# muonzoo/cutesdr

Measured on AMD Instinct MI355X. Metric: complex IQ MSamples/s through CFastFIR+demod chain; achieved HBM GB/s vs peak, higher is better.
Workload: dtype f32; 1 GPU; C3: 256 channels/GPU x 2^19 IQ samples, 16384-pt CFastFIR overlap-save (8193 taps, hop 8192), shared -5..+5 kHz filter @62.5 kS/s; channels_per_gpu=256, samples_per_channel=524288, fft_size=16384, parallelism=channels sharded x1, no data-path collective

## Files before the change

cutesdr_amd/csrc/capi_fastfir.hip:

```cpp
#include "capi_common.hpp"
#include "capi_internal.hpp"
#include <algorithm>
#include "fastfir_kernels.h"
#include "fastfir_design_kernels.h"
#include "host_math.hpp"
#include "patch_queue.hpp"
#include <cmath>
#include <cstdlib>
#include <cstring>
#include <vector>

using namespace csdr;

static int log2_of(int n)
{
    int l = 0;
    while ((1 << l) < n) l++;
    return ((1 << l) == n) ? l : -1;
}

struct csdr_fastfir_batch {
    int device, channels, n, log2n;
    int cus;
    hipStream_t last_stream;
// ... 60 lines not shown
            if (e == hipSuccess) e = hipEventRecord(b->ev_design, s);
        }
    }
    const int rr = b->patches.retire(s);
    if (rc) return rc;
    if (e != hipSuccess) return fail(CSDR_EHIP, "filter design launch: %s", hipGetErrorString(e));
    return rr;
}

static int fetch_mirror(csdr_fastfir_batch *b, int slot)
{
    if (!b->stale[slot]) return CSDR_OK;
    const int rc = flush_control(b, b->last_stream);
    if (rc) return rc;
    if (b->ev_design) CSDR_HIP(hipEventSynchronize(b->ev_design));
    CSDR_HIP(hipMemcpy(b->resp[slot].data(), b->d_resp + (size_t)slot * 2 * b->n, sizeof(cd) * (size_t)b->n, hipMemcpyDeviceToHost));
    b->stale[slot] = 0;
    return CSDR_OK;
}

static int design_state(csdr_fastfir_batch *b)
{
    if (b->d_resp) return CSDR_OK;
    const size_t n = (size_t)b->n, p = n / 2 + 1;
    const auto win = fastfir_window((int)p);
    const auto tw = design_twiddles(n);
    if (!b->d_win) CSDR_HIP(hipMalloc((void **)&b->d_win, p * sizeof(double)));
    if (!b->d_tw) CSDR_HIP(hipMalloc((void **)&b->d_tw, n * sizeof(double)));
    if (!b->d_perm) CSDR_HIP(hipMalloc((void **)&b->d_perm, n * sizeof(int)));
    if (!b->d_perm2) CSDR_HIP(hipMalloc((void **)&b->d_perm2, n * sizeof(int)));
    if (!b->d_permg) CSDR_HIP(hipMalloc((void **)&b->d_permg, n * sizeof(int)));
    CSDR_HIP(hipMemcpy(b->d_win, win->data(), p * sizeof(double), hipMemcpyHostToDevice));
    CSDR_HIP(hipMemcpy(b->d_tw, tw.data(), n * sizeof(double), hipMemcpyHostToDevice));
    CSDR_HIP(hipMemcpy(b->d_perm, b->perm.data(), n * sizeof(int), hipMemcpyHostToDevice));
    CSDR_HIP(hipMemcpy(b->d_perm2, b->perm2.data(), n * sizeof(int), hipMemcpyHostToDevice));
    CSDR_HIP(hipMemcpy(b->d_permg, b->permg.data(), n * sizeof(int), hipMemcpyHostToDevice));
    CSDR_HIP(hipMalloc((void **)&b->d_resp, (size_t)b->channels * n * sizeof(cd)));
    return CSDR_OK;
}

static void build_perm(csdr_fastfir_batch *b)
{
    const int T = b->n / 32;
    b->perm.resize(b->n);
    for (int j = 0; j < 16; j++)
        for (int t = 0; t < T; t++)
            for (int e = 0; e < 2; e++)
                b->perm[(j * T + t) * 2 + e] = fastfir_bin_of(b->log2n, t, 2 * j + e);
    b->perm2.clear();
    {
        b->perm2.resize(b->n);
        for (int j = 0; j < 16; j++)
            for (int t = 0; t < T; t++)
                for (int e = 0; e < 2; e++) b->perm2[(j * T + t) * 2 + e] = fastfir2_bin_of(b->log2n, t, j, e);
    }
    b->permg.resize(b->n);
    for (int i = 0; i < 8; i++)
        for (int t = 0; t < T; t++)
            for (int c = 0; c < 4; c++) b->permg[(i * T + t) * 4 + c] = fastfir2_gain_bin_of(b->log2n, t, i, c);
}

static int upload_response(csdr_fastfir_batch *b, int slot, const std::vector<cd> &H)
{
    std::vector<float> dev(2 * (size_t)b->n);
    for (int pass = 0; pass < 2; pass++) {
        const std::vector<int> &perm = pass ? b->perm2 : b->perm;
        float *dst = pass ? b->d_h2 : b->d_h;
        if (perm.empty() || !dst) continue;
        for (int i = 0; i < b->n; i++) {
            const cd v = H[perm[i]];
            dev[2 * i] = (float)v.real();
            dev[2 * i + 1] = (float)v.imag();
        }
        const int rc = b->patches.add(dst + (size_t)slot * 2 * b->n, dev.data(), dev.size() * sizeof(float));
        if (rc) return rc;
    }
    for (int i = 0; i < b->n; i++) dev[i] = (float)fastfir_gain(H[b->permg[i]], b->permg[i]);
    return b->patches.add(b->d_gain + (size_t)slot * b->n, dev.data(), (size_t)b->n * sizeof(float));
}

static int set_response(csdr_fastfir_batch *b, int slot, const std::vector<cd> &H)
{
    cancel_job(b, slot);
    const int rc = upload_response(b, slot, H);
    if (rc) return rc;
    b->resp[slot] = H;
    b->stale[slot] = 0;
    return CSDR_OK;
}

extern "C" {

csdr_fastfir_batch *csdr_fastfir_batch_create(int device, int channels, int fft_size)
{
    const int l2 = log2_of(fft_size);
    if (l2 < 11 || l2 > 14 || channels < 1) {
        fail(CSDR_EINVAL, "fft_size must be 2048..16384 (power of two), channels >= 1");
        return nullptr;
    }
    if (!device_ok(device)) return nullptr;
    csdr_fastfir_batch *b = new csdr_fastfir_batch();
    b->device = device; b->channels = channels; b->n = fft_size; b->log2n = l2;
    b->per_channel = false; b->hist_cur = 0; b->dbg_stage = 0; b->dbg_out = nullptr;
    b->last_stream = nullptr;
    {
        int cus = 0;
        if (hipDeviceGetAttribute(&cus, hipDeviceAttributeMultiprocessorCount, device) != hipSuccess || cus <= 0) cus = 256;
        b->cus = cus;
    }
    {
        const char *v = getenv("CSDR_FASTFIR_VARIANT");
        b->variant = (v && atoi(v) == 0) ? 0 : 2;
// ... 358 lines not shown
```

cutesdr_amd/csrc/capi_hosttest.hip:

```cpp
#include "capi_common.hpp"
#include "host_math.hpp"
#include "dc_host.hpp"
#include "pc_host.hpp"
#include "display_plan.hpp"
#include "testgen_host.hpp"
#include "scope_host.hpp"
#include "fastfir_kernels.h"
#include "fft_core.hpp"
#include <cstring>

using namespace csdr;

template <int SIGN> static void host_head4_gain(const float *x4, const float *g4, float *out4)
{
    v2f x[4];
    for (int q = 0; q < 4; q++) x[q] = v2f{x4[2 * q], x4[2 * q + 1]};
    dit_head4_gain<0, 4, SIGN>(x, v2f{g4[0], g4[1]}, v2f{g4[2], g4[3]});
    for (int q = 0; q < 4; q++) { out4[2 * q] = x[q].x; out4[2 * q + 1] = x[q].y; }
}
template <int R, int SIGN> static void host_dft_middle(const float *in, float *out)
{
    v2f x[R];
    for (int n = 0; n < R; n++) x[bitrev<R>(n)] = v2f{in[2 * n], in[2 * n + 1]};
    static_for<0, R / 4>([&](auto G) { dit_head4<G.value, R, SIGN>(x); });
    if constexpr (R == 32) dit_single<8, 32, SIGN>(x);
    static_for<0, R / 4>([&](auto I) { dit_tail_middle<I.value, R, SIGN>(x); });
    for (int r = 0; r < R / 2; r++) { out[2 * r] = x[R / 4 + r].x; out[2 * r + 1] = x[R / 4 + r].y; }
}

extern "C" {

int csdr__host_fastfir_design(int n, double flo, double fhi, double off, double fs, double *h_out)
{
    std::vector<cd> H;
    if (!fastfir_design(n, flo, fhi, off, fs, H)) return -1;
    memcpy(h_out, H.data(), sizeof(cd) * n);
    return 0;
}
int csdr__host_design_job(double flo, double fhi, double off, double fs, double *nfc, double *nfs)
{
    return fastfir_design_job(flo, fhi, off, fs, *nfc, *nfs) ? 0 : -1;
}
int csdr__host_fastfir_bin_of(int log2n, int t, int r) { return fastfir_bin_of(log2n, t, r); }
int csdr__host_fastfir_gains(int n, double flo, double fhi, double off, double fs, double *h_out, double *p_out)
{
    std::vector<cd> H;
    if (!fastfir_design(n, flo, fhi, off, fs, H)) return -1;
    memcpy(h_out, H.data(), sizeof(cd) * n);
    for (int k = 0; k < n; k++) p_out[k] = fastfir_gain(H[k], k);
    return 0;
}
int csdr__host_fastfir2_bin_of(int log2n, int t, int j, int e) { return fastfir2_bin_of(log2n, t, j, e); }
int csdr__host_fastfir2_gain_bin_of(int log2n, int t, int i, int c) { return fastfir2_gain_bin_of(log2n, t, i, c); }

void csdr__host_dit_head4_gain(int sign, const float *x4, const float *g4, float *out4)
{
    if (sign > 0) host_head4_gain<+1>(x4, g4, out4); else host_head4_gain<-1>(x4, g4, out4);
}
int csdr__host_dft_middle(int r, int sign, const float *in, float *out)
{
    if (r == 16 && sign > 0) host_dft_middle<16, +1>(in, out);
    else if (r == 16) host_dft_middle<16, -1>(in, out);
    else if (r == 32 && sign > 0) host_dft_middle<32, +1>(in, out);
    else if (r == 32) host_dft_middle<32, -1>(in, out);
    else return -1;
    return 0;
}

int csdr__host_dc_plan(double in_rate, double bw, int *codes, double *out_rate, int *warmup)
{
    DcPlan p = dc_make_plan(in_rate, bw);
    for (int i = 0; i < p.nstages; i++) codes[i] = p.kind[i];
    *out_rate = p.out_rate; *warmup = p.W;
    return p.nstages;
}
int csdr__host_dc_stage_taps(double in_rate, double bw, int s, double *h)
{
    DcPlan p = dc_make_plan(in_rate, bw);
    if (s < 0 || s >= p.nstages) return -1;
    const DcStage &st = p.st[s];
    const int L = st.hist + (p.kind[s] == 3 ? 2 : 1);
    for (int i = 0; i < L; i++) h[i] = 0;
    if (st.center >= 0) h[st.center] = st.ccoef;
    for (int q = 0; q < st.npairs; q++) { h[st.a[q]] = st.c[q]; h[st.b[q]] = st.c[q]; }
    return L;
}
void csdr__host_dc_nco(double freq, double cw, double in_rate, unsigned long long *inc, double *stored)
{
    DcHostChan c;
    c.in_rate = in_rate; c.cw_offset = cw;
    c.set_frequency(freq);
    *inc = c.inc; *stored = c.nco_freq;
}
int csdr__host_fir_design(int kind, double scale, double astop, double fpass, double fstop, double fs,
                          double hilbert_off, double *coef, double *icoef, double *qcoef)
{
    HostFir f;
    if (kind == 0) f.init_lp(scale, astop, fpass, fstop, fs);
    else f.init_hp(scale, astop, fpass, fstop, fs);
    if (hilbert_off != 0.0) f.gen_hilbert(hilbert_off);
    for (int i = 0; i < f.ntaps; i++) { coef[i] = f.coef[i]; icoef[i] = f.icoef[i]; qcoef[i] = f.qcoef[i]; }
    return f.ntaps;
}
void csdr__host_iir_design(int kind, double f0, double q, double fs, double *c5)
{
    PcIir f;
// ... 185 lines not shown
```

cutesdr_amd/csrc/fastfir2_kernels.hip:

```cpp
#define CSDR_FMA_BFLY 1
#define CSDR_PLAIN_CONST_FMA 1
#include "launch_once.hpp"
#include "fastfir_dev.hpp"
#include "fastfir_kernels.h"

namespace csdr {

#define CSDR_SB() __builtin_amdgcn_sched_barrier(0)

#ifndef K1_LDAUX
#define K1_LDAUX 2
#endif
#ifndef K1_STAUX
#define K1_STAUX 2
#endif
#ifndef K1_HREG
#define K1_HREG 8
#endif
#ifndef K1_REALGAIN
#define K1_REALGAIN 1
#endif
#ifndef K1_TWREG
#define K1_TWREG 0
#endif
#ifndef K1_HREG4K
#define K1_HREG4K 4
#endif
#ifndef K1_W1_FETCH_MAX_R0
#define K1_W1_FETCH_MAX_R0 2
#endif
#ifndef K1_HREG2K
#define K1_HREG2K 8
#endif

#ifdef CSDR_K1_STAMPS
#define CSDR_STAMP(i)                                                                         \
    do {                                                                                      \
        CSDR_SB();                                                                            \
        unsigned long long now_;                                                              \
        asm volatile("s_memtime %0\n\ts_waitcnt lgkmcnt(0)" : "=s"(now_)::"memory");         \
        CSDR_SB();                                                                            \
        acc_[i] += now_ - last_;                                                              \
        last_ = now_;                                                                         \
    } while (0)
#else
#define CSDR_STAMP(i) do { } while (0)
#endif

#define CSDR_PRIO(p) __builtin_amdgcn_s_setprio(p)

#ifdef K1_ABLATE
__device__ __forceinline__ void keep_alive(v4f v) { asm volatile("" ::"v"(v)); }
#endif

template <int LOG2N>
struct K1Cfg {
    using Base = FastFirCfg<LOG2N>;
    static constexpr int VW = LOG2N == 12 ? 2 : (LOG2N == 11 ? 4 : 1);
    static constexpr int TV = Base::T;
    static constexpr int T = VW * TV;
    static constexpr int LDS_BYTES = (VW * Base::LDS_DATA + 1024) * 8;
};

template <int LOG2N, bool RG>
__device__ __forceinline__ void fastfir_os2_body(const FastFirArgs a)
{
    CSDR_WG_TRACE_SCOPE(a.trace, WGT_FF);
    static_assert(!RG || LOG2N == 14, "the quarter-block shift is whole rows of the outer pass at N = 16384 only");
    using Cfg = FastFirCfg<LOG2N>;
    constexpr int N = Cfg::N, T = Cfg::T, R0 = Cfg::R0, G = Cfg::G, L = N / 2;
    constexpr int HALF = R0 / 2;
    constexpr int VW = K1Cfg<LOG2N>::VW;
    constexpr int HREG = RG ? 0 : (LOG2N == 12 ? K1_HREG4K : (LOG2N == 11 ? K1_HREG2K : K1_HREG));
    constexpr int TWREG = RG ? K1_TWREG : 0;
    static_assert(R0 == 16 || R0 == 8 || R0 == 4 || R0 == 2, "the grouped outer pass is written for N = 2048 ... 16384");
    auto block_barrier = [] {
        if constexpr (LOG2N == 11) {
            __builtin_amdgcn_fence(__ATOMIC_RELEASE, "wavefront"); __builtin_amdgcn_wave_barrier(); __builtin_amdgcn_fence(__ATOMIC_ACQUIRE, "wavefront");
        } else {
            __syncthreads();
        }
    };
    extern __shared__ __attribute__((aligned(16))) unsigned char smem_raw[];
    const int t = VW == 1 ? (int)threadIdx.x : (int)threadIdx.x % T, vw = VW == 1 ? 0 : (int)threadIdx.x / T;
    v2f *lds = reinterpret_cast<v2f *>(smem_raw) + vw * Cfg::LDS_DATA;
    v2f *tw2 = reinterpret_cast<v2f *>(smem_raw) + VW * Cfg::LDS_DATA;
    if constexpr (VW > 1) {
        for (int i = threadIdx.x; i < 1024; i += VW * T) tw2[i] = a.tw2[i];
        __syncthreads();
    }

    int wg = blockIdx.x * VW + vw, ch, run;
    if ((a.channels & 7) == 0) {
        int xcd = wg & 7, slot = wg >> 3;
        ch = (slot / a.runs) * 8 + xcd;
        run = slot % a.runs;
    } else {
        ch = wg / a.runs;
        run = wg % a.runs;
    }
    const int b0 = run * a.blocks_per_run;
    int b1 = b0 + a.blocks_per_run;
    if (b1 > a.nblocks) b1 = a.nblocks;
#if defined(__HIP_DEVICE_COMPILE__) && !defined(__gfx950__)
#error "fastfir_os2_kernel<12> relies on gfx950's s_barrier ignoring terminated waves (two virtual workgroups per workgroup)"
#endif
    if (ch >= a.channels || b0 >= b1) return;

    if constexpr (VW == 1)
        for (int i = t; i < 1024; i += T) tw2[i] = a.tw2[i];

    const rsrc_t r_in = make_rsrc(a.in + (long)ch * a.in_stride, (unsigned)a.nblocks * L * 8u);
    const rsrc_t r_hist = make_rsrc(a.hist + (long)ch * L, L * 8u);
    const rsrc_t r_out = make_rsrc(a.out + (long)ch * a.out_stride, (unsigned)a.nblocks * L * 8u);
    const rsrc_t r_h = make_rsrc(a.h + (long)ch * a.h_stride, N * 8u);
    const rsrc_t r_g = make_rsrc(a.gain + (long)ch * (a.h_stride / 2), N * 4u);
    constexpr int PSTEP = 2 * T, PSTEP_LDS = PSTEP + 2 * (PSTEP / 32), PSTEP_B = PSTEP * 8;
    const int voff = t * 16;
    auto load_half = [&](rsrc_t r, int soff, v2f (&dst)[16]) {
#pragma unroll
        for (int n1 = 0; n1 < HALF; n1++)
#pragma unroll
            for (int pp = 0; pp < G / 2; pp++) {
                v4f v = buf_load16_aux<K1_LDAUX>(r, voff + pp * PSTEP_B, soff + n1 * 8192);
                dst[(2 * pp) * HALF + n1] = v2f{v.x, v.y};
                dst[(2 * pp + 1) * HALF + n1] = v2f{v.z, v.w};
            }
    };

    constexpr bool W1_RESIDENT = R0 > K1_W1_FETCH_MAX_R0;
    auto w_pair = [&](int pp) { return *reinterpret_cast<const v4f *>(a.tw1 + PSTEP * pp + 2 * t); };
    v2f w1[R0 > 2 ? G : 1];
    auto load_w1 = [&] {
        if constexpr (R0 > 2) {
#pragma unroll
            for (int pp = 0; pp < G / 2; pp++) { const v4f v = w_pair(pp); w1[2 * pp] = v2f{v.x, v.y}; w1[2 * pp + 1] = v2f{v.z, v.w}; }
        }
    };
    load_w1();
    v2f pw[G][R0];
    if constexpr (R0 > 2) {
#pragma unroll
        for (int e = 0; e < G; e++) twiddle_powers<R0>(opaque(w1[e]), pw[e]);
    }

    v4f hv[RG ? 1 : 16];
#pragma unroll
    for (int j = 0; j < HREG; j++) hv[j] = buf_load16(r_h, t * 16, j * (T * 16));
    v4f pv[RG ? 8 : 1];
    if constexpr (RG) {
#pragma unroll
        for (int i = 0; i < 8; i++) pv[i] = buf_load16(r_g, t * 16, i * (T * 16));
    }
#ifdef K1_ABLATE
    v4f habl = {1.0f, 0.0f, 1.0f, 0.0f};
    asm volatile("" : "+v"(habl));
    v2f twabl = {0.8f, 0.6f};
    asm volatile("" : "+v"(twabl));
#endif
    v2f x[32];
    v2f hp[16], hq[16];

    if (b0 == 0) load_half(r_hist, 0, hp);
    else load_half(r_in, (b0 - 1) * (L * 8), hp);
    load_half(r_in, b0 * (L * 8), hq);

    const int sb = t >> 5, sn = t & 31;
    v2f *const col = lds + lds_pad(1024 * sb) + sn;
    const v2f *const twc = tw2 + sn;
    v2f twr[TWREG > 0 ? TWREG : 1];
#pragma unroll
    for (int k1 = 1; k1 <= TWREG; k1++) twr[k1 - 1] = a.tw2[32 * k1 + sn];
    auto pass_tw = [&](auto K1) {
        constexpr int k1 = K1.value;
        if constexpr (k1 <= TWREG) return twr[k1 - 1];
        else return lds_ld8(twc + 32 * k1);
    };
    v2f *const rowp = lds + 34 * t;
    v2f *const outer = lds + lds_pad(2 * t);
    constexpr int OUTER_ROW = 1024 + 2 * (1024 / 32);

#ifdef K1_CYC
    const unsigned long long cyc0_ = __builtin_amdgcn_s_memtime(), rt0_ = __builtin_amdgcn_s_memrealtime();
#endif
#ifdef CSDR_K1_STAMPS
    unsigned long long acc_[16] = {0, 0, 0, 0, 0, 0, 0, 0, 0, 0, 0, 0, 0, 0, 0, 0}, last_;
    asm volatile("s_memtime %0\n\ts_waitcnt lgkmcnt(0)" : "=s"(last_)::"memory");
#endif
    auto one_block = [&](const int b, v2f (&oldh)[16], v2f (&newh)[16]) {
        CSDR_SB();
        CSDR_PRIO(1);
        {
            v2f y[G][R0];
            static_for<0, HALF>([&](auto N1) {
                static_for<0, G>([&](auto E) {
                    constexpr int e = E.value, n1 = N1.value, po = bitrev<R0>(n1), pn = bitrev<R0>(HALF + n1);
                    y[e][po] = oldh[e * HALF + n1]; y[e][pn] = newh[e * HALF + n1];
                });
            });
            if constexpr (R0 == 2) {
                static_for<0, G>([&](auto E) { bfly_dit<0, +1>(y[E.value][0], y[E.value][1]); });
            } else {
                static_for<0, (R0 >= 8 ? R0 / 4 : 1)>([&](auto Gg) {
                    static_for<0, G>([&](auto E) { dit_head4<Gg.value, R0, +1>(y[E.value]); });
                });
            }
            CSDR_SB();
            load_half(r_in, (b + 1 < a.nblocks ? b + 1 : a.nblocks - 1) * (L * 8), oldh);
            CSDR_SB();
            CSDR_PRIO(0);
            v4f wv[16];
            if constexpr (R0 == 16) {
                static_for<0, R0 / 4 + 1>([&](auto Ii) {
                    constexpr int i = Ii.value;
                    if constexpr (i < R0 / 4) {
                        dit_tail<i, R0, +1>(y[0]);
                        dit_tail<i, R0, +1>(y[1]);
                        static_for<0, 4>([&](auto P) {
                            constexpr int k0 = i + 4 * P.value;
                            if constexpr (k0 != 0) {
                                y[0][k0] = cmul(y[0][k0], pw[0][k0]);
                                y[1][k0] = cmul(y[1][k0], pw[1][k0]);
                            }
                            wv[k0] = store_operand(y[0][k0], y[1][k0]);
                        });
                    }
                    if constexpr (i > 0) {
                        CSDR_STORE_GROUP_BEGIN();
                        static_for<0, 4>([&](auto P) {
                            constexpr int k0 = (i - 1) + 4 * P.value;
                            *reinterpret_cast<v4f *>(outer + OUTER_ROW * k0) = wv[k0];
                        });
                        CSDR_STORE_GROUP_END();
                    } else {
                        CSDR_SB();
                    }
                });
            } else if constexpr (R0 == 2) {
                v4f wq[8];
                static_for<0, 8>([&](auto PP) { wq[PP.value] = w_pair(PP.value); });
                static_for<0, 5>([&](auto Ii) {
                    constexpr int i = Ii.value;
                    if constexpr (i < 4) {
                        static_for<0, 2>([&](auto Q) {
                            constexpr int pp = 2 * i + Q.value;
                            y[2 * pp][1] = cmul(y[2 * pp][1], v2f{wq[pp].x, wq[pp].y});
                            y[2 * pp + 1][1] = cmul(y[2 * pp + 1][1], v2f{wq[pp].z, wq[pp].w});
                            wv[pp] = store_operand(y[2 * pp][0], y[2 * pp + 1][0]);
                            wv[8 + pp] = store_operand(y[2 * pp][1], y[2 * pp + 1][1]);
                        });
                    }
                    if constexpr (i > 0) {
                        CSDR_STORE_GROUP_BEGIN();
                        static_for<0, 2>([&](auto Q) {
                            constexpr int pp = 2 * (i - 1) + Q.value;
                            *reinterpret_cast<v4f *>(outer + PSTEP_LDS * pp) = wv[pp];
                            *reinterpret_cast<v4f *>(outer + OUTER_ROW + PSTEP_LDS * pp) = wv[8 + pp];
                        });
                        CSDR_STORE_GROUP_END();
                    } else {
                        CSDR_SB();
                    }
                });
            } else {
                constexpr int NG = 4, RPG = R0 / NG;
                static_for<0, NG + 1>([&](auto Ii) {
                    constexpr int i = Ii.value;
                    if constexpr (i < NG) {
                        if constexpr (R0 == 8)
                            static_for<0, G>([&](auto E) { bfly_dit<4 * i, +1>(y[E.value][i], y[E.value][i + 4]); });
                        static_for<0, RPG>([&](auto P) {
                            constexpr int k0 = i + NG * P.value;
                            static_for<0, G>([&](auto E) {
                                if constexpr (k0 != 0) y[E.value][k0] = cmul(y[E.value][k0], pw[E.value][k0]);
                            });
                            static_for<0, G / 2>([&](auto PP) {
                                wv[k0 * (G / 2) + PP.value] = store_operand(y[2 * PP.value][k0], y[2 * PP.value + 1][k0]);
                            });
                        });
                    }
                    if constexpr (i > 0) {
                        CSDR_STORE_GROUP_BEGIN();
                        static_for<0, RPG>([&](auto P) {
                            constexpr int k0 = (i - 1) + NG * P.value;
                            static_for<0, G / 2>([&](auto PP) {
                                *reinterpret_cast<v4f *>(outer + OUTER_ROW * k0 + PSTEP_LDS * PP.value) = wv[k0 * (G / 2) + PP.value];
                            });
                        });
                        CSDR_STORE_GROUP_END();
                    } else {
                        CSDR_SB();
                    }
                });
            }
        }
        CSDR_STAMP(0);
#ifdef ABL_BAR
        __builtin_amdgcn_fence(__ATOMIC_RELEASE, "wavefront"); __builtin_amdgcn_wave_barrier(); __builtin_amdgcn_fence(__ATOMIC_ACQUIRE, "wavefront");
#else
        block_barrier();
#endif
        CSDR_STAMP(1);

        CSDR_PRIO(3);
        {
            auto fetch = [&](auto Gg) {
                static_for<0, 4>([&](auto Q) {
                    constexpr int p = 4 * Gg.value + Q.value;
                    x[p] = lds_ld8(col + 34 * bitrev<32>(p));
                });
            };
            static_for<0, 3>(fetch);
            CSDR_SB();
            static_for<0, 8>([&](auto Gg) {
                if constexpr (Gg.value + 3 < 8) fetch(std::integral_constant<int, Gg.value + 3>{});
                dit_head4<Gg.value, 32, +1>(x);
                if constexpr ((Gg.value & 1) == 1) CSDR_SB();
            });
            CSDR_STAMP(7);
            dit_single<8, 32, +1>(x);
            CSDR_SB();
            v2f tw[2][4];
#ifdef ABL_TW
            static_for<1, 4>([&](auto P) { tw[0][P.value] = twabl; });
#else
            static_for<1, 4>([&](auto P) { tw[0][P.value] = pass_tw(std::integral_constant<int, 8 * P.value>{}); });
#endif
            CSDR_SB();
            CSDR_STAMP(8);
            static_for<0, 9>([&](auto Ii) {
                constexpr int i = Ii.value;
                if constexpr (i < 7)
#ifdef ABL_TW
                    static_for<0, 4>([&](auto P) { tw[(i + 1) & 1][P.value] = twabl; });
#else
                    static_for<0, 4>([&](auto P) { tw[(i + 1) & 1][P.value] = pass_tw(std::integral_constant<int, i + 1 + 8 * P.value>{}); });
#endif
                if constexpr (i < 8) {
#ifdef ABL_H
                    if constexpr (!RG) { hv[2 * i] = habl; hv[2 * i + 1] = habl; }
#else
                    if constexpr (!RG && 2 * i >= HREG) hv[2 * i] = buf_load16(r_h, t * 16, (2 * i) * (T * 16));
                    if constexpr (!RG && 2 * i + 1 >= HREG) hv[2 * i + 1] = buf_load16(r_h, t * 16, (2 * i + 1) * (T * 16));
#endif
                    dit_tail<i, 32, +1>(x);
                    static_for<0, 4>([&](auto P) {
                        constexpr int k1 = i + 8 * P.value;
                        if constexpr (k1 != 0) x[k1] = cmul(x[k1], tw[i & 1][P.value]);
                    });
                }
                if constexpr (i > 0)
                    static_for<0, 4>([&](auto P) {
                        constexpr int k1 = (i - 1) + 8 * P.value;
                        lds_st8(col + 34 * k1, x[k1]);
                    });
                CSDR_SB();
            });
        }
        CSDR_STAMP(2);
        __builtin_amdgcn_fence(__ATOMIC_RELEASE, "wavefront");
        __builtin_amdgcn_wave_barrier();
        __builtin_amdgcn_fence(__ATOMIC_ACQUIRE, "wavefront");

        CSDR_PRIO(2);
        {
            v2f y[32];
            static_for<0, 4>([&](auto Q) {
                static_for<0, 4>([&](auto P) {
                    constexpr int j = Q.value + 4 * P.value;
                    const v4f v = *reinterpret_cast<const v4f *>(rowp + 2 * j);
                    x[bitrev<32>(2 * j)] = v2f{v.x, v.y};
                    x[bitrev<32>(2 * j + 1)] = v2f{v.z, v.w};
                });
            });
            CSDR_SB();
            static_for<0, 4>([&](auto Q) {
                dit_head4<bitrev<8>(2 * Q.value), 32, +1>(x);
                dit_head4<bitrev<8>(2 * Q.value + 1), 32, +1>(x);
                CSDR_SB();
            });
            dit_single<8, 32, +1>(x);
            CSDR_SB();
            static_for<0, 8>([&](auto Ii) {
                constexpr int i = Ii.value, g = bitrev<8>(i);
                dit_tail<i, 32, +1>(x);
                y[4 * g] = x[i]; y[4 * g + 1] = x[i + 16]; y[4 * g + 2] = x[i + 8]; y[4 * g + 3] = x[i + 24];
                if constexpr (RG)
                    dit_head4_gain<g, 32, -1>(y, v2f{pv[i].x, pv[i].y}, v2f{pv[i].z, pv[i].w});
                else
                    dit_head4_tw<g, 32, -1>(y, v2f{hv[2 * i].x, hv[2 * i].y}, v2f{hv[2 * i].z, hv[2 * i].w},
                                            v2f{hv[2 * i + 1].x, hv[2 * i + 1].y}, v2f{hv[2 * i + 1].z, hv[2 * i + 1].w});
                if constexpr ((i & 1) == 1) CSDR_SB();
            });
#pragma unroll
            for (int i = 0; i < 32; i++) x[i] = y[i];
            CSDR_PRIO(1);
            dit_single<8, 32, -1>(x);
            CSDR_SB();
            v4f wv[16];
            static_for<0, 5>([&](auto Q) {
                constexpr int q = Q.value;
                if constexpr (q < 4) {
                    dit_tail<2 * q, 32, -1>(x);
                    dit_tail<2 * q + 1, 32, -1>(x);
                    static_for<0, 4>([&](auto P) {
                        constexpr int j = q + 4 * P.value;
                        wv[j] = store_operand(x[2 * j], x[2 * j + 1]);
                    });
                }
                if constexpr (q > 0) {
                    CSDR_STORE_GROUP_BEGIN();
                    static_for<0, 4>([&](auto P) {
                        constexpr int j = (q - 1) + 4 * P.value;
                        *reinterpret_cast<v4f *>(rowp + 2 * j) = wv[j];
                    });
                    CSDR_STORE_GROUP_END();
                } else {
                    CSDR_SB();
                }
            });
        }
        CSDR_STAMP(3);
        __builtin_amdgcn_fence(__ATOMIC_RELEASE, "wavefront");
        __builtin_amdgcn_wave_barrier();
        __builtin_amdgcn_fence(__ATOMIC_ACQUIRE, "wavefront");

        CSDR_PRIO(0);
        {
            v2f tw[32];
            auto fetch = [&](auto Gg) {
                static_for<0, 4>([&](auto Q) {
                    constexpr int r = 4 * Gg.value + Q.value;
                    x[r] = lds_ld8(col + 34 * bitrev<32>(r));
                });
                static_for<0, 4>([&](auto Q) {
                    constexpr int r = 4 * Gg.value + Q.value;
#ifdef ABL_TW
                    if constexpr (r != 0) tw[r] = twabl;
#else
                    if constexpr (r != 0) tw[r] = pass_tw(std::integral_constant<int, bitrev<32>(r)>{});
#endif
                });
            };
            static_for<0, 2>(fetch);
            CSDR_SB();
            static_for<0, 8>([&](auto Gg) {
                constexpr int g = Gg.value;
                if constexpr (g + 2 < 8) fetch(std::integral_constant<int, g + 2>{});
                dit_head4_conjtw<g, 32, -1, g == 0>(x, tw[4 * g], tw[4 * g + 1], tw[4 * g + 2], tw[4 * g + 3]);
                if constexpr ((g & 1) == 1) CSDR_SB();
            });
            dit_single<8, 32, -1>(x);
            CSDR_SB();
            static_for<0, 9>([&](auto I) {
                constexpr int i = I.value;
                if constexpr (i < 8) dit_tail<i, 32, -1>(x);
                if constexpr (i > 0)
                    static_for<0, 4>([&](auto P) {
                        constexpr int n1 = (i - 1) + 8 * P.value;
                        lds_st8(col + 34 * n1, x[n1]);
                    });
                CSDR_SB();
            });
        }
        CSDR_STAMP(4);
#ifdef ABL_BAR
        __builtin_amdgcn_fence(__ATOMIC_RELEASE, "wavefront"); __builtin_amdgcn_wave_barrier(); __builtin_amdgcn_fence(__ATOMIC_ACQUIRE, "wavefront");
#else
        block_barrier();
#endif
        CSDR_STAMP(5);

        CSDR_PRIO(3);
        {
            v2f y[G][R0];
            static_for<0, R0>([&](auto Rr) {
                constexpr int r = Rr.value, k0 = bitrev<R0>(r);
                static_for<0, G / 2>([&](auto PP) {
                    const v4f v = *reinterpret_cast<const v4f *>(outer + OUTER_ROW * k0 + PSTEP_LDS * PP.value);
                    y[2 * PP.value][r] = v2f{v.x, v.y};
                    y[2 * PP.value + 1][r] = v2f{v.z, v.w};
                });
            });
            if constexpr (R0 > 2) {
                if constexpr (!W1_RESIDENT) load_w1();
#pragma unroll
                for (int e = 0; e < G; e++) twiddle_powers<R0>(opaque(w1[e]), pw[e]);
                CSDR_SB();
                static_for<0, (R0 >= 8 ? R0 / 4 : 1)>([&](auto Gg) {
                    constexpr int g = Gg.value;
                    static_for<0, G>([&](auto E) {
                        constexpr int e = E.value;
                        dit_head4_conjtw<g, R0, -1, g == 0>(y[e], pw[e][bitrev<R0>(4 * g)], pw[e][bitrev<R0>(4 * g + 1)],
                                                            pw[e][bitrev<R0>(4 * g + 2)], pw[e][bitrev<R0>(4 * g + 3)]);
                    });
                    if constexpr ((g & 1) == 1) CSDR_SB();
                });
            }
            CSDR_PRIO(2);
            v4f sv[8];
            if constexpr (R0 == 16) {
                static_for<0, R0 / 4 + 1>([&](auto I) {
                    constexpr int i = I.value;
                    if constexpr (i < R0 / 4) {
                        if constexpr (RG) {
                            dit_tail_middle<i, R0, -1>(y[0]);
                            dit_tail_middle<i, R0, -1>(y[1]);
                            sv[2 * i] = store_operand(y[0][i + 4], y[1][i + 4]);
                            sv[2 * i + 1] = store_operand(y[0][i + 8], y[1][i + 8]);
                        } else {
                            dit_tail_upper<i, R0, -1>(y[0]);
                            dit_tail_upper<i, R0, -1>(y[1]);
                            sv[2 * i] = store_operand(y[0][i + 8], y[1][i + 8]);
                            sv[2 * i + 1] = store_operand(y[0][i + 12], y[1][i + 12]);
                        }
                    }
                    if constexpr (i > 0) {
                        CSDR_STORE_GROUP_BEGIN();
#ifdef ABL_GST
                        keep_alive(sv[2 * (i - 1)]); keep_alive(sv[2 * (i - 1) + 1]);
#else
                        buf_store16_aux<K1_STAUX>(r_out, voff, b * (L * 8) + (i - 1) * 8192, sv[2 * (i - 1)]);
                        buf_store16_aux<K1_STAUX>(r_out, voff, b * (L * 8) + (i - 1 + 4) * 8192, sv[2 * (i - 1) + 1]);
#endif
                        CSDR_STORE_GROUP_END();
                    } else {
                        CSDR_SB();
                    }
                });
            } else if constexpr (R0 == 2) {
                v4f wq[8];
                static_for<0, 8>([&](auto PP) { wq[PP.value] = w_pair(PP.value); });
                static_for<0, 5>([&](auto I) {
                    constexpr int i = I.value;
                    if constexpr (i < 4) {
                        static_for<0, 2>([&](auto Q) {
                            constexpr int pp = 2 * i + Q.value;
                            const v2f d0 = y[2 * pp][0] - cmul_conj(y[2 * pp][1], v2f{wq[pp].x, wq[pp].y});
                            const v2f d1 = y[2 * pp + 1][0] - cmul_conj(y[2 * pp + 1][1], v2f{wq[pp].z, wq[pp].w});
                            sv[pp] = store_operand(d0, d1);
                        });
                    }
                    if constexpr (i > 0) {
                        CSDR_STORE_GROUP_BEGIN();
                        static_for<0, 2>([&](auto Q) {
// ... 78 lines not shown
    fastfir_os2_body<LOG2N, LOG2N == 14 && K1_REALGAIN>(a);
}
__global__ __launch_bounds__(K1Cfg<14>::T) __attribute__((amdgpu_waves_per_eu(2, 2)))
void fastfir_os2h_kernel(FastFirArgs a)
{
    fastfir_os2_body<14, false>(a);
}

template <int LOG2N>
static hipError_t launch2_one(const FastFirArgs &a, hipStream_t stream, int *which)
{
    using Cfg = K1Cfg<LOG2N>;
    void (*kernel)(FastFirArgs) = &fastfir_os2_kernel<LOG2N>;
    if (LOG2N == 14 && !(K1_REALGAIN && a.gain)) kernel = &fastfir_os2h_kernel;
    if (which) *which = (LOG2N == 14 && K1_REALGAIN && kernel != &fastfir_os2h_kernel) ? FASTFIR_KERNEL_PIPELINED_GAIN : FASTFIR_KERNEL_PIPELINED_H;
    hipError_t e = kernel == &fastfir_os2h_kernel ? CSDR_MAX_LDS_ONCE(&fastfir_os2h_kernel, Cfg::LDS_BYTES)
                                                  : CSDR_MAX_LDS_ONCE(&fastfir_os2_kernel<LOG2N>, Cfg::LDS_BYTES);
    if (e != hipSuccess) return e;
#ifdef CSDR_WG_TRACE
    FastFirArgs b = a;
    b.trace = wgtrace_next();
    hipLaunchKernelGGL(kernel, dim3((a.channels * a.runs + Cfg::VW - 1) / Cfg::VW), dim3(Cfg::T), Cfg::LDS_BYTES, stream, b);
    return hipGetLastError();
#endif
    hipLaunchKernelGGL(kernel, dim3((a.channels * a.runs + Cfg::VW - 1) / Cfg::VW), dim3(Cfg::T), Cfg::LDS_BYTES, stream, a);
    return hipGetLastError();
}

hipError_t fastfir2_launch(int log2n, const FastFirArgs &a, hipStream_t stream, int *kernel)
{
    switch (log2n) {
    case 11: return launch2_one<11>(a, stream, kernel);
    case 12: return launch2_one<12>(a, stream, kernel);
    case 13: return launch2_one<13>(a, stream, kernel);
    case 14: return launch2_one<14>(a, stream, kernel);
    default: return hipErrorInvalidValue;
    }
}

int fastfir2_twreg() { return K1_TWREG; }

int fastfir2_bin_of(int log2n, int t, int j, int e)
{
    const int R0 = (1 << log2n) / 1024;
    const int i = j >> 1, h = j & 1;
    const int k2 = i + 8 * h + 16 * e;
    return (t >> 5) + R0 * ((t & 31) + 32 * k2);
}
int fastfir2_gain_bin_of(int log2n, int t, int i, int c)
{
    return fastfir2_bin_of(log2n, t, 2 * i + (c >> 1), c & 1);
}

}
```

cutesdr_amd/csrc/fastfir_kernels.h:

```cpp
#pragma once
#include <hip/hip_runtime.h>
#include "wg_trace.hpp"

namespace csdr {

typedef float v2f_h __attribute__((ext_vector_type(2)));
typedef float v4f_h __attribute__((ext_vector_type(4)));

struct FastFirArgs {
    const v2f_h *in;
    const v2f_h *hist;
    v2f_h *hist_next;
    v2f_h *out;
    const v4f_h *h;
    const v4f_h *gain;
    const v2f_h *tw1;
    const v2f_h *tw2;
    long in_stride;
    long out_stride;
    long h_stride;
    int channels;
    int nblocks;
    int blocks_per_run;
    int runs;
    int dbg_stage;
    v2f_h *dbg;
#ifdef CSDR_WG_TRACE
    WgTraceArg trace;
#endif
};

hipError_t fastfir_launch(int log2n, const FastFirArgs &a, hipStream_t stream);
int fastfir_bin_of(int log2n, int t, int r);

enum FastFirKernel { FASTFIR_KERNEL_NONE = -1, FASTFIR_KERNEL_GENERIC = 0, FASTFIR_KERNEL_PIPELINED_H = 1, FASTFIR_KERNEL_PIPELINED_GAIN = 2 };
hipError_t fastfir2_launch(int log2n, const FastFirArgs &a, hipStream_t stream, int *kernel = nullptr);
int fastfir2_twreg();
int fastfir2_bin_of(int log2n, int t, int j, int e);
int fastfir2_gain_bin_of(int log2n, int t, int i, int c);

}
```

cutesdr_amd/csrc/fft_core.hpp:

```cpp
#pragma once
#include <hip/hip_runtime.h>

namespace csdr {

typedef float v2f __attribute__((ext_vector_type(2)));
typedef float v4f __attribute__((ext_vector_type(4)));

static constexpr float kCos32[32] = {
    1.0f, 0.98078528040323044913f, 0.92387953251128675613f, 0.83146961230254523708f,
    0.70710678118654752440f, 0.55557023301960222474f, 0.38268343236508977173f, 0.19509032201612826785f,
    0.0f, -0.19509032201612826785f, -0.38268343236508977173f, -0.55557023301960222474f,
    -0.70710678118654752440f, -0.83146961230254523708f, -0.92387953251128675613f, -0.98078528040323044913f,
    -1.0f, -0.98078528040323044913f, -0.92387953251128675613f, -0.83146961230254523708f,
    -0.70710678118654752440f, -0.55557023301960222474f, -0.38268343236508977173f, -0.19509032201612826785f,
    0.0f, 0.19509032201612826785f, 0.38268343236508977173f, 0.55557023301960222474f,
    0.70710678118654752440f, 0.83146961230254523708f, 0.92387953251128675613f, 0.98078528040323044913f};

#if defined(__HIP_DEVICE_COMPILE__) && !defined(CSDR_NO_PK_ASM)
#define CSDR_PK_ASM 1
#else
#define CSDR_PK_ASM 0
#endif

__host__ __device__ __forceinline__ v2f cmul_c(v2f a, v2f w)
// ... 222 lines not shown
        });
    });
}
template <int LEN, int R, int SIGN>
__host__ __device__ __forceinline__ void dit_single(v2f (&x)[R])
{
    constexpr int H = LEN / 2;
    static_for<0, R / LEN>([&](auto B) {
        static_for<0, H>([&](auto I) {
            constexpr int a = B.value * LEN + I.value, b = a + H;
            bfly_dit<I.value *(32 / LEN), SIGN>(x[a], x[b]);
        });
    });
}
template <int I, int R, int SIGN>
__host__ __device__ __forceinline__ void dif_head(v2f (&x)[R])
{
    static_assert(R >= 8 && I < R / 4, "dif_head");
    constexpr int Q = R / 4;
    bfly_dif<I *(32 / R), SIGN>(x[I], x[I + 2 * Q]);
    bfly_dif<(I + Q) * (32 / R), SIGN>(x[I + Q], x[I + 3 * Q]);
    bfly_dif<I *(64 / R), SIGN>(x[I], x[I + Q]);
    bfly_dif<I *(64 / R), SIGN>(x[I + 2 * Q], x[I + 3 * Q]);
}
template <int G, int R, int SIGN>
__host__ __device__ __forceinline__ void dif_tail4(v2f (&x)[R])
{
    constexpr int a = 4 * G;
    bfly_dif<0, SIGN>(x[a], x[a + 2]);
    bfly_dif<8, SIGN>(x[a + 1], x[a + 3]);
    bfly_dif<0, SIGN>(x[a], x[a + 1]);
    bfly_dif<0, SIGN>(x[a + 2], x[a + 3]);
}
template <int G, int R, int SIGN>
__host__ __device__ __forceinline__ void dit_head4(v2f (&x)[R])
{
    constexpr int a = 4 * G;
    bfly_dit<0, SIGN>(x[a], x[a + 1]);
    bfly_dit<0, SIGN>(x[a + 2], x[a + 3]);
    bfly_dit<0, SIGN>(x[a], x[a + 2]);
    bfly_dit<8, SIGN>(x[a + 1], x[a + 3]);
}
template <int G, int R, int SIGN, bool FIRST_PLAIN>
__host__ __device__ __forceinline__ void dit_head4_conjtw(v2f (&x)[R], v2f t0, v2f t1, v2f t2, v2f t3)
{
    constexpr int a = 4 * G;
    if constexpr (!FIRST_PLAIN) x[a] = cmul_conj(x[a], t0);
    x[a + 2] = cmul_conj(x[a + 2], t2);
    bfly_fma_conj(x[a], x[a + 1], t1);
    bfly_fma_conj(x[a + 2], x[a + 3], t3);
    bfly_dit<0, SIGN>(x[a], x[a + 2]);
    bfly_dit<8, SIGN>(x[a + 1], x[a + 3]);
}
template <int G, int R, int SIGN>
__host__ __device__ __forceinline__ void dit_head4_tw(v2f (&x)[R], v2f t0, v2f t1, v2f t2, v2f t3)
{
    constexpr int a = 4 * G;
    x[a] = cmul(x[a], t0);
    x[a + 2] = cmul(x[a + 2], t2);
    bfly_fma(x[a], x[a + 1], t1);
    bfly_fma(x[a + 2], x[a + 3], t3);
    bfly_dit<0, SIGN>(x[a], x[a + 2]);
    bfly_dit<8, SIGN>(x[a + 1], x[a + 3]);
}
__host__ __device__ __forceinline__ void bfly_gain(v2f &xa, v2f &xb, v2f g)
{
#if CSDR_PK_ASM
    v2f t, a, b;
    asm("v_pk_mul_f32 %0, %1, %2 op_sel:[0,0] op_sel_hi:[1,0]" : "=v"(t) : "v"(xa), "v"(g));
    asm("v_pk_fma_f32 %0, %1, %2, %3 op_sel:[0,1,0] op_sel_hi:[1,1,1]" : "=v"(a) : "v"(xb), "v"(g), "v"(t));
    asm("v_pk_fma_f32 %0, %1, %2, %3 op_sel:[0,1,0] op_sel_hi:[1,1,1] neg_lo:[0,1,0] neg_hi:[0,1,0]"
        : "=v"(b) : "v"(xb), "v"(g), "v"(t));
    xa = a; xb = b;
#else
    const v2f t = xa * g.xx, v = xb * g.yy;
    xa = t + v; xb = t - v;
#endif
}
template <int G, int R, int SIGN>
__host__ __device__ __forceinline__ void dit_head4_gain(v2f (&x)[R], v2f g01, v2f g23)
{
    constexpr int a = 4 * G;
    bfly_gain(x[a], x[a + 1], g01);
    bfly_gain(x[a + 2], x[a + 3], g23);
    bfly_dit<0, SIGN>(x[a], x[a + 2]);
    bfly_dit<8, SIGN>(x[a + 1], x[a + 3]);
}
template <int K, int SIGN>
__host__ __device__ __forceinline__ void bfly_dit_sum(v2f &xa, const v2f xb)
{
    if constexpr (K == 0) {
        xa = xa + xb;
    } else if constexpr (K == 8) {
        xa = add_jv<SIGN>(xa, xb);
    } else {
        constexpr float c = kCos32[K];
        constexpr float s = (SIGN > 0 ? 1.0f : -1.0f) * kCos32[(K + 24) & 31];
        const v2f w1 = {c, s}, w2 = {-s, c};
        const v2f t = __builtin_elementwise_fma(xb.xx, w1, xa);
        xa = __builtin_elementwise_fma(xb.yy, w2, t);
    }
}
template <int K, int SIGN>
__host__ __device__ __forceinline__ void bfly_dit_lower(const v2f xa, v2f &xb)
{
    if constexpr (K == 0) {
// ... 76 lines not shown
```

Before: 216,700 MSamples/s.

## Share conjugate-symmetric twiddles across FFT passes and reorder bins by slot

```diff
diff --git a/cutesdr_amd/csrc/capi_fastfir.hip b/cutesdr_amd/csrc/capi_fastfir.hip
--- a/cutesdr_amd/csrc/capi_fastfir.hip
+++ b/cutesdr_amd/csrc/capi_fastfir.hip
@@ -136,12 +136,12 @@
         b->perm2.resize(b->n);
         for (int j = 0; j < 16; j++)
             for (int t = 0; t < T; t++)
-                for (int e = 0; e < 2; e++) b->perm2[(j * T + t) * 2 + e] = fastfir2_bin_of(b->log2n, t, j, e);
+                for (int e = 0; e < 2; e++) b->perm2[(j * T + t) * 2 + e] = fastfir2_slot_bin(b->log2n, t, j, e);
     }
     b->permg.resize(b->n);
     for (int i = 0; i < 8; i++)
         for (int t = 0; t < T; t++)
-            for (int c = 0; c < 4; c++) b->permg[(i * T + t) * 4 + c] = fastfir2_gain_bin_of(b->log2n, t, i, c);
+            for (int c = 0; c < 4; c++) b->permg[(i * T + t) * 4 + c] = fastfir2_gain_slot_bin(b->log2n, t, i, c);
 }
 
 static int upload_response(csdr_fastfir_batch *b, int slot, const std::vector<cd> &H)
diff --git a/cutesdr_amd/csrc/capi_hosttest.hip b/cutesdr_amd/csrc/capi_hosttest.hip
--- a/cutesdr_amd/csrc/capi_hosttest.hip
+++ b/cutesdr_amd/csrc/capi_hosttest.hip
@@ -52,6 +52,10 @@
 }
 int csdr__host_fastfir2_bin_of(int log2n, int t, int j, int e) { return fastfir2_bin_of(log2n, t, j, e); }
 int csdr__host_fastfir2_gain_bin_of(int log2n, int t, int i, int c) { return fastfir2_gain_bin_of(log2n, t, i, c); }
+int csdr__host_fastfir2_slot_bin(int log2n, int t, int j, int e) { return fastfir2_slot_bin(log2n, t, j, e); }
+int csdr__host_fastfir2_gain_slot_bin(int log2n, int t, int i, int c) { return fastfir2_gain_slot_bin(log2n, t, i, c); }
+void csdr__host_fastfir2_twshare_shift(int log2n, int t, int *inner, int *outer) { fastfir2_twshare_shift(log2n, t, inner, outer); }
+int csdr__host_fastfir2_twshare(void) { return fastfir2_twshare(); }
 
 void csdr__host_dit_head4_gain(int sign, const float *x4, const float *g4, float *out4)
 {
diff --git a/cutesdr_amd/csrc/fastfir2_kernels.hip b/cutesdr_amd/csrc/fastfir2_kernels.hip
--- a/cutesdr_amd/csrc/fastfir2_kernels.hip
+++ b/cutesdr_amd/csrc/fastfir2_kernels.hip
@@ -20,8 +20,11 @@
 #ifndef K1_REALGAIN
 #define K1_REALGAIN 1
 #endif
+#ifndef K1_TWSHARE
+#define K1_TWSHARE 2
+#endif
 #ifndef K1_TWREG
-#define K1_TWREG 0
+#define K1_TWREG (K1_TWSHARE >= 2 ? 16 : 0)
 #endif
 #ifndef K1_HREG4K
 #define K1_HREG4K 4
@@ -53,6 +56,32 @@
 __device__ __forceinline__ void keep_alive(v4f v) { asm volatile("" ::"v"(v)); }
 #endif
 
+constexpr int tws_group(int step) { return step < 2 ? 4 * step : ((step & 1) ? 8 - step / 2 : step / 2); }
+constexpr int tws_set(int step) { return step < 2 ? step : 1 + step / 2; }
+constexpr bool tws_opens(int step) { return step < 2 || (step & 1) == 0; }
+constexpr int tws_row(int set, int slot)
+{
+    if (set < 2) return slot < 2 ? 8 - 4 * set + 8 * slot : 0;
+    const int m = set - 1;
+    return slot == 0 ? m : (slot == 1 ? m + 8 : (slot == 2 ? 8 - m : 16 - m));
+}
+constexpr int tws_row_of(int k1) { return k1 <= 16 ? k1 : 32 - k1; }
+constexpr int tws_set_of(int k1)
+{
+    const int r = tws_row_of(k1) & 7;
+    return r == 0 ? 0 : (r == 4 ? 1 : 1 + (r < 4 ? r : 8 - r));
+}
+constexpr int tws_slot_of(int k1)
+{
+    for (int slot = 0; slot < 4; slot++)
+        if (tws_row(tws_set_of(k1), slot) == tws_row_of(k1)) return slot;
+    return -1;
+}
+static_assert(K1_TWSHARE >= 0 && K1_TWSHARE <= 2 && K1_TWREG >= 0 && K1_TWREG <= (K1_TWSHARE ? 16 : 31), "K1_TWSHARE / K1_TWREG");
+static_assert(tws_group(2) == 1 && tws_group(3) == 7 && tws_group(7) == 5 && tws_set(7) == 4 && tws_set_of(31) == 2 &&
+              tws_slot_of(24) == 0 && tws_slot_of(16) == 1 && tws_slot_of(20) == 1 && tws_slot_of(25) == 2 && tws_slot_of(23) == 1,
+              "twiddle sets of K1_TWSHARE");
+
 template <int LOG2N>
 struct K1Cfg {
     using Base = FastFirCfg<LOG2N>;
@@ -72,6 +101,7 @@
     constexpr int HALF = R0 / 2;
     constexpr int VW = K1Cfg<LOG2N>::VW;
     constexpr int HREG = RG ? 0 : (LOG2N == 12 ? K1_HREG4K : (LOG2N == 11 ? K1_HREG2K : K1_HREG));
+    constexpr bool TWS = K1_TWSHARE >= 1 && LOG2N == 14;
     constexpr int TWREG = RG ? K1_TWREG : 0;
     static_assert(R0 == 16 || R0 == 8 || R0 == 4 || R0 == 2, "the grouped outer pass is written for N = 2048 ... 16384");
     auto block_barrier = [] {
@@ -138,10 +168,12 @@
         }
     };
     load_w1();
-    v2f pw[G][R0];
+    constexpr bool OUTER_SHARE = K1_TWSHARE >= 2 && R0 == 16;
+    constexpr int PWN = OUTER_SHARE ? R0 / 2 + 1 : R0;
+    v2f pw[G][PWN];
     if constexpr (R0 > 2) {
 #pragma unroll
-        for (int e = 0; e < G; e++) twiddle_powers<R0>(opaque(w1[e]), pw[e]);
+        for (int e = 0; e < G; e++) twiddle_powers<PWN>(opaque(w1[e]), pw[e]);
     }
 
     v4f hv[RG ? 1 : 16];
@@ -218,7 +250,10 @@
                         dit_tail<i, R0, +1>(y[1]);
                         static_for<0, 4>([&](auto P) {
                             constexpr int k0 = i + 4 * P.value;
-                            if constexpr (k0 != 0) {
+                            if constexpr (OUTER_SHARE && k0 > R0 / 2) {
+                                y[0][k0] = cmul_conj(y[0][k0], pw[0][R0 - k0]);
+                                y[1][k0] = cmul_conj(y[1][k0], pw[1][R0 - k0]);
+                            } else if constexpr (k0 != 0) {
                                 y[0][k0] = cmul(y[0][k0], pw[0][k0]);
                                 y[1][k0] = cmul(y[1][k0], pw[1][k0]);
                             }
@@ -320,6 +355,47 @@
             CSDR_STAMP(7);
             dit_single<8, 32, +1>(x);
             CSDR_SB();
+            if constexpr (TWS) {
+            v2f tw[5][4];
+            auto load_set = [&](auto S) {
+                static_for<0, 4>([&](auto Q) {
+                    constexpr int row = tws_row(S.value, Q.value);
+#ifdef ABL_TW
+                    if constexpr (row != 0) tw[S.value][Q.value] = twabl;
+#else
+                    if constexpr (row != 0) tw[S.value][Q.value] = pass_tw(std::integral_constant<int, row>{});
+#endif
+                });
+            };
+            load_set(std::integral_constant<int, 0>{});
+            CSDR_SB();
+            CSDR_STAMP(8);
+            static_for<0, 9>([&](auto St) {
+                constexpr int s = St.value;
+                if constexpr (s < 7 && tws_opens(s + 1)) load_set(std::integral_constant<int, tws_set(s + 1)>{});
+                if constexpr (s < 8) {
+                    constexpr int i = tws_group(s);
+#ifdef ABL_H
+                    if constexpr (!RG) { hv[2 * s] = habl; hv[2 * s + 1] = habl; }
+#else
+                    if constexpr (!RG && 2 * s >= HREG) hv[2 * s] = buf_load16(r_h, t * 16, (2 * s) * (T * 16));
+                    if constexpr (!RG && 2 * s + 1 >= HREG) hv[2 * s + 1] = buf_load16(r_h, t * 16, (2 * s + 1) * (T * 16));
+#endif
+                    dit_tail<i, 32, +1>(x);
+                    static_for<0, 4>([&](auto P) {
+                        constexpr int k1 = i + 8 * P.value;
+                        if constexpr (k1 != 0 && k1 <= 16) x[k1] = cmul(x[k1], tw[tws_set_of(k1)][tws_slot_of(k1)]);
+                        if constexpr (k1 > 16) x[k1] = cmul_conj(x[k1], tw[tws_set_of(k1)][tws_slot_of(k1)]);
+                    });
+                }
+                if constexpr (s > 0)
+                    static_for<0, 4>([&](auto P) {
+                        constexpr int k1 = tws_group(s - 1) + 8 * P.value;
+                        lds_st8(col + 34 * k1, x[k1]);
+                    });
+                CSDR_SB();
+            });
+            } else {
             v2f tw[2][4];
 #ifdef ABL_TW
             static_for<1, 4>([&](auto P) { tw[0][P.value] = twabl; });
@@ -356,6 +432,7 @@
                     });
                 CSDR_SB();
             });
+            }
         }
         CSDR_STAMP(2);
         __builtin_amdgcn_fence(__ATOMIC_RELEASE, "wavefront");
@@ -427,6 +504,36 @@
 
         CSDR_PRIO(0);
         {
+            if constexpr (TWS) {
+            v2f tw[5][4];
+            auto fetch = [&](auto St) {
+                constexpr int s = St.value, g = bitrev<8>(tws_group(s));
+                static_for<0, 4>([&](auto Q) {
+                    constexpr int r = 4 * g + Q.value;
+                    x[r] = lds_ld8(col + 34 * bitrev<32>(r));
+                });
+                if constexpr (tws_opens(s))
+                    static_for<0, 4>([&](auto Q) {
+                        constexpr int row = tws_row(tws_set(s), Q.value);
+#ifdef ABL_TW
+                        if constexpr (row != 0) tw[tws_set(s)][Q.value] = twabl;
+#else
+                        if constexpr (row != 0) tw[tws_set(s)][Q.value] = pass_tw(std::integral_constant<int, row>{});
+#endif
+                    });
+            };
+            static_for<0, 2>(fetch);
+            CSDR_SB();
+            static_for<0, 8>([&](auto St) {
+                constexpr int s = St.value, i = tws_group(s), g = bitrev<8>(i);
+                if constexpr (s + 2 < 8) fetch(std::integral_constant<int, s + 2>{});
+                constexpr int ka = i == 0 ? 8 : i, kb = i + 16, kc = i + 8, kd = i + 24;
+                dit_head4_seltw<g, 32, -1, i == 0, (ka <= 16), (kb <= 16), (kc <= 16), (kd <= 16)>(
+                    x, tw[tws_set_of(ka)][tws_slot_of(ka)], tw[tws_set_of(kb)][tws_slot_of(kb)],
+                    tw[tws_set_of(kc)][tws_slot_of(kc)], tw[tws_set_of(kd)][tws_slot_of(kd)]);
+                if constexpr ((s & 1) == 1) CSDR_SB();
+            });
+            } else {
             v2f tw[32];
             auto fetch = [&](auto Gg) {
                 static_for<0, 4>([&](auto Q) {
@@ -450,6 +557,7 @@
                 dit_head4_conjtw<g, 32, -1, g == 0>(x, tw[4 * g], tw[4 * g + 1], tw[4 * g + 2], tw[4 * g + 3]);
                 if constexpr ((g & 1) == 1) CSDR_SB();
             });
+            }
             dit_single<8, 32, -1>(x);
             CSDR_SB();
             static_for<0, 9>([&](auto I) {
@@ -485,12 +593,19 @@
             if constexpr (R0 > 2) {
                 if constexpr (!W1_RESIDENT) load_w1();
 #pragma unroll
-                for (int e = 0; e < G; e++) twiddle_powers<R0>(opaque(w1[e]), pw[e]);
+                for (int e = 0; e < G; e++) twiddle_powers<PWN>(opaque(w1[e]), pw[e]);
                 CSDR_SB();
                 static_for<0, (R0 >= 8 ? R0 / 4 : 1)>([&](auto Gg) {
                     constexpr int g = Gg.value;
                     static_for<0, G>([&](auto E) {
                         constexpr int e = E.value;
+                        if constexpr (OUTER_SHARE) {
+                            constexpr int ka = bitrev<R0>(4 * g), kb = bitrev<R0>(4 * g + 1), kc = bitrev<R0>(4 * g + 2), kd = bitrev<R0>(4 * g + 3);
+                            constexpr int H0 = R0 / 2;
+                            dit_head4_seltw<g, R0, -1, g == 0, (ka <= H0), (kb <= H0), (kc <= H0), (kd <= H0)>(
+                                y[e], pw[e][ka <= H0 ? ka : R0 - ka], pw[e][kb <= H0 ? kb : R0 - kb],
+                                pw[e][kc <= H0 ? kc : R0 - kc], pw[e][kd <= H0 ? kd : R0 - kd]);
+                        } else
                         dit_head4_conjtw<g, R0, -1, g == 0>(y[e], pw[e][bitrev<R0>(4 * g)], pw[e][bitrev<R0>(4 * g + 1)],
                                                             pw[e][bitrev<R0>(4 * g + 2)], pw[e][bitrev<R0>(4 * g + 3)]);
                     });
@@ -675,4 +790,24 @@
     return fastfir2_bin_of(log2n, t, 2 * i + (c >> 1), c & 1);
 }
 
-}
+int fastfir2_twshare() { return K1_TWSHARE; }
+void fastfir2_twshare_shift(int log2n, int t, int *inner, int *outer)
+{
+    *inner = (K1_TWSHARE >= 1 && log2n == 14 && (t & 31) >= 17) ? 1 : 0;
+    *outer = (K1_TWSHARE >= 2 && log2n == 14 && (t >> 5) > 8) ? 1 : 0;
+}
+int fastfir2_slot_bin(int log2n, int t, int j, int e)
+{
+    const int R0 = (1 << log2n) / 1024;
+    int inner, outer;
+    fastfir2_twshare_shift(log2n, t, &inner, &outer);
+    const int k2 = ((j >> 1) + 8 * (j & 1) + 16 * e - inner) & 31;
+    const int sub = ((t & 31) + 32 * k2 - outer) & 1023;
+    return (t >> 5) + R0 * sub;
+}
+int fastfir2_gain_slot_bin(int log2n, int t, int i, int c)
+{
+    return fastfir2_slot_bin(log2n, t, 2 * i + (c >> 1), c & 1);
+}
+
+}
diff --git a/cutesdr_amd/csrc/fastfir_kernels.h b/cutesdr_amd/csrc/fastfir_kernels.h
--- a/cutesdr_amd/csrc/fastfir_kernels.h
+++ b/cutesdr_amd/csrc/fastfir_kernels.h
@@ -38,5 +38,9 @@
 int fastfir2_twreg();
 int fastfir2_bin_of(int log2n, int t, int j, int e);
 int fastfir2_gain_bin_of(int log2n, int t, int i, int c);
+int fastfir2_twshare();
+void fastfir2_twshare_shift(int log2n, int t, int *inner, int *outer);
+int fastfir2_slot_bin(int log2n, int t, int j, int e);
+int fastfir2_gain_slot_bin(int log2n, int t, int i, int c);
 
 }
diff --git a/cutesdr_amd/csrc/fft_core.hpp b/cutesdr_amd/csrc/fft_core.hpp
--- a/cutesdr_amd/csrc/fft_core.hpp
+++ b/cutesdr_amd/csrc/fft_core.hpp
@@ -298,6 +298,17 @@
     bfly_dit<0, SIGN>(x[a], x[a + 2]);
     bfly_dit<8, SIGN>(x[a + 1], x[a + 3]);
 }
+template <int G, int R, int SIGN, bool FIRST_PLAIN, bool C0, bool C1, bool C2, bool C3>
+__host__ __device__ __forceinline__ void dit_head4_seltw(v2f (&x)[R], v2f t0, v2f t1, v2f t2, v2f t3)
+{
+    constexpr int a = 4 * G;
+    if constexpr (!FIRST_PLAIN) x[a] = C0 ? cmul_conj(x[a], t0) : cmul(x[a], t0);
+    x[a + 2] = C2 ? cmul_conj(x[a + 2], t2) : cmul(x[a + 2], t2);
+    if constexpr (C1) bfly_fma_conj(x[a], x[a + 1], t1); else bfly_fma(x[a], x[a + 1], t1);
+    if constexpr (C3) bfly_fma_conj(x[a + 2], x[a + 3], t3); else bfly_fma(x[a + 2], x[a + 3], t3);
+    bfly_dit<0, SIGN>(x[a], x[a + 2]);
+    bfly_dit<8, SIGN>(x[a + 1], x[a + 3]);
+}
 template <int G, int R, int SIGN>
 __host__ __device__ __forceinline__ void dit_head4_tw(v2f (&x)[R], v2f t0, v2f t1, v2f t2, v2f t3)
 {
```

Result: faster. 226,100 MSamples/s (median of 6 runs) (+4.3%).
